# hassony2/handobjectconsist

Hardware: AMD Instinct MI355X
Metric: trainmeshwarp iters/sec (render+warp, B=64, 256x256) (higher is better)
Workload: dtype f32; 1 GPU; trainmeshwarp.py consist step, per-GPU B=64, 256x256, hand 778v/1552f + object 1002v/2000f (7104 faces after fill-back), ResNet-18 fp32 (MIOpen convolutions, channels-last, + fused HIP BatchNorm/ReLU/residual/max-pool kernels), Adam; global_batch=64, image_size=256, parallelism=dp1

## Files before the change

handobjectconsist_amd/csrc/stem_wrw.hip:

```cpp
#include "bn_device.hpp"

namespace mr {

constexpr int SW_TY = 4, SW_TX = 32;
constexpr int SW_BLOCKS = 512;
constexpr int SW_C = 64;
constexpr int SW_TAPS = 7 * 7 * 3;
constexpr int SW_NB = 5;
constexpr int SW_OUT = SW_C * SW_TAPS;
constexpr int SW_PH = 2 * SW_TY + 5;
constexpr int SW_PROW = (2 * SW_TX + 5) * 3;
constexpr int SW_PW = 213;
constexpr int SW_G = SW_TY * SW_TX * SW_C;
constexpr int SW_LDS = SW_G + SW_PH * SW_PW;
constexpr int SW_FIN_RUNS = 8, SW_FIN_RUN = SW_BLOCKS / SW_FIN_RUNS;
static_assert(SW_LDS >= SW_C * SW_NB * 32, "the wave reduction reuses the tile's LDS");
static_assert(SW_OUT % 32 == 0, "finish kernel: 32 outputs per workgroup");

typedef float f32x16 __attribute__((ext_vector_type(16)));

struct WrwParams {
    const float* grad_y;
    const float* grad_y2;
    const float* rec_d;
    const unsigned char* rec_code;
    BnAffine bn;
    const float* image;
    float* partial;
    int N, Hin, Win, H, W, OH, OW;
    int tiles_x, tiles_y;
    int64_t tiles;
};

__device__ __forceinline__ void wrw_keep(float& v) { asm volatile("" : "+v"(v)); }
__device__ __forceinline__ void wrw_keep(unsigned& v) { asm volatile("" : "+v"(v)); }
__device__ __forceinline__ void wrw_keep(float4& v) { asm volatile("" : "+v"(v.x), "+v"(v.y), "+v"(v.z), "+v"(v.w)); }

__global__ __launch_bounds__(256, 2) void stem_conv_wrw_kernel(WrwParams p) {
    __shared__ __attribute__((aligned(16))) float lds[SW_LDS];
    float* const G = lds;
    float* const patch = lds + SW_G;
    const int tid = threadIdx.x, lane = tid & 63, wave = tid >> 6, half = lane >> 5, l31 = lane & 31;

    const int c0 = 4 * (tid & 15), qcol = tid >> 4;
    float a[4], b[4];
#pragma unroll
    for (int i = 0; i < 4; i++) {
        float mean;
        channel_consts(p.bn, c0 + i, mean, a[i], b[i]);
    }

    const float* aptr[2];
    const float* bptr[SW_NB];
#pragma unroll
    for (int m = 0; m < 2; m++) aptr[m] = G + (wave * SW_TX + 16 * half) * SW_C + ((l31 + 32 * m) ^ (32 * half));
#pragma unroll
    for (int n = 0; n < SW_NB; n++) {
        const int t = l31 + 32 * n;
        const int off = t < SW_TAPS ? (t / 21) * SW_PW + t % 21 : 0;
        bptr[n] = patch + 2 * wave * SW_PW + 6 * 16 * half + off;
    }

    f32x16 acc[2][SW_NB];
#pragma unroll
    for (int m = 0; m < 2; m++)
#pragma unroll
        for (int n = 0; n < SW_NB; n++)
#pragma unroll
            for (int r = 0; r < 16; r++) acc[m][n][r] = 0.0f;

    const int per_image = p.tiles_x * p.tiles_y;
    for (int64_t tile = blockIdx.x; tile < p.tiles; tile += gridDim.x) {
        const int n = (int)(tile / per_image), rem = (int)(tile - (int64_t)n * per_image);
        const int cy0 = (rem / p.tiles_x) * SW_TY, cx0 = (rem % p.tiles_x) * SW_TX;

        {
            const int iy0 = 2 * cy0 - 3, ix0 = 2 * cx0 - 3;
            const int c = tid < SW_PROW ? tid : SW_PROW - 1, ix = ix0 + c / 3;
            const bool col = ix >= 0 && ix < p.Win;
            const float* src = p.image + (int64_t)n * p.Hin * p.Win * 3 + (col ? ix0 * 3 + c : 0);
            float pv[SW_PH];
#pragma unroll
            for (int r = 0; r < SW_PH; r++) {
                const int iy = iy0 + r, iyc = iy < 0 ? 0 : (iy >= p.Hin ? p.Hin - 1 : iy);
                pv[r] = src[(int64_t)iyc * p.Win * 3];
            }
#pragma unroll
            for (int r = 0; r < SW_PH; r++) wrw_keep(pv[r]);
#pragma unroll
            for (int r = 0; r < SW_PH; r++) {
                const int iy = iy0 + r;
                if (!col || iy < 0 || iy >= p.Hin) pv[r] = 0.0f;
            }
            if (tid < SW_PROW) {
#pragma unroll
                for (int r = 0; r < SW_PH; r++) patch[r * SW_PW + tid] = pv[r];
            }
        }

#pragma unroll 1
        for (int qr = 0; qr < SW_TY / 2; qr++) {
            float s[2][2][4];
            unsigned code[2][2][4];
            unsigned idw[2][2];
            float4 dv[2][2], g1[2][2], g2[2][2];
#pragma unroll
            for (int j = 0; j < 2; j++)
#pragma unroll
                for (int k = 0; k < 2; k++) {
                    const int wy = (cy0 >> 1) + qr + j, wx = (cx0 >> 1) + qcol + k;
                    const int64_t o = (((int64_t)n * p.OH + (wy < p.OH ? wy : p.OH - 1)) * p.OW + (wx < p.OW ? wx : p.OW - 1)) * SW_C + c0;
                    idw[j][k] = *reinterpret_cast<const unsigned*>(p.rec_code + o);
                    dv[j][k] = *reinterpret_cast<const float4*>(p.rec_d + o);
                    g1[j][k] = *reinterpret_cast<const float4*>(p.grad_y + o);
                    g2[j][k] = *reinterpret_cast<const float4*>((p.grad_y2 ? p.grad_y2 : p.grad_y) + o);
                }
#pragma unroll
            for (int j = 0; j < 2; j++)
#pragma unroll
                for (int k = 0; k < 2; k++) { wrw_keep(idw[j][k]); wrw_keep(dv[j][k]); wrw_keep(g1[j][k]); wrw_keep(g2[j][k]); }
#pragma unroll
            for (int j = 0; j < 2; j++)
#pragma unroll
                for (int k = 0; k < 2; k++) {
                    const int wy = (cy0 >> 1) + qr + j, wx = (cx0 >> 1) + qcol + k;
                    const bool win = wy < p.OH && wx < p.OW;
                    const float d[4] = {dv[j][k].x, dv[j][k].y, dv[j][k].z, dv[j][k].w};
                    const float gv[4] = {p.grad_y2 ? g1[j][k].x + g2[j][k].x : g1[j][k].x, p.grad_y2 ? g1[j][k].y + g2[j][k].y : g1[j][k].y,
                                         p.grad_y2 ? g1[j][k].z + g2[j][k].z : g1[j][k].z, p.grad_y2 ? g1[j][k].w + g2[j][k].w : g1[j][k].w};
#pragma unroll
                    for (int i = 0; i < 4; i++) {
                        code[j][k][i] = win ? (idw[j][k] >> (8 * i)) & 255u : 255u;
                        s[j][k][i] = (d[i] * a[i] + b[i] > 0.0f) ? gv[i] : 0.0f;
                    }
                }
#pragma unroll
            for (int pr = 0; pr < 2; pr++)
#pragma unroll
                for (int pc = 0; pc < 2; pc++) {
                    const int py = 2 * qr + pr, px = 2 * qcol + pc;
                    float g[4] = {0.0f, 0.0f, 0.0f, 0.0f};
#pragma unroll
                    for (int dy = 0; dy < 2; dy++) {
                        const int j = pr - dy, kh = pr + 1 - 2 * j;
                        if (j < 0) continue;
#pragma unroll
                        for (int dx = 0; dx < 2; dx++) {
                            const int k = pc - dx, kw = pc + 1 - 2 * k;
                            if (k < 0) continue;
                            const unsigned want = (unsigned)(kh * 3 + kw);
#pragma unroll
                            for (int i = 0; i < 4; i++) g[i] += code[j][k][i] == want ? s[j][k][i] : 0.0f;
                        }
                    }
                    const bool in = cy0 + py < p.H && cx0 + px < p.W;
                    float4 out;
                    out.x = in ? g[0] * a[0] : 0.0f; out.y = in ? g[1] * a[1] : 0.0f;
                    out.z = in ? g[2] * a[2] : 0.0f; out.w = in ? g[3] * a[3] : 0.0f;
                    *reinterpret_cast<float4*>(G + (py * SW_TX + px) * SW_C + (c0 ^ (((px >> 4) & 1) << 5))) = out;
                }
        }
        __syncthreads();

#pragma unroll
        for (int s = 0; s < 16; s++) {
            float av[2], bv[SW_NB];
#pragma unroll
            for (int m = 0; m < 2; m++) av[m] = aptr[m][s * SW_C];
#pragma unroll
            for (int nb = 0; nb < SW_NB; nb++) bv[nb] = bptr[nb][6 * s];
#pragma unroll
            for (int m = 0; m < 2; m++)
#pragma unroll
                for (int nb = 0; nb < SW_NB; nb++)
                    acc[m][nb] = __builtin_amdgcn_mfma_f32_32x32x2f32(av[m], bv[nb], acc[m][nb], 0, 0, 0);
        }
        __syncthreads();
    }

#pragma unroll 1
    for (int w = 0; w < 4; w++) {
        if (wave == w) {
#pragma unroll
            for (int m = 0; m < 2; m++)
#pragma unroll
                for (int nb = 0; nb < SW_NB; nb++)
#pragma unroll
                    for (int r = 0; r < 16; r++) {
                        float* const slot = lds + ((m * SW_NB + nb) * 16 + r) * 64 + lane;
                        *slot = w > 0 ? *slot + acc[m][nb][r] : acc[m][nb][r];
                    }
        }
        __syncthreads();
    }
    float* const out = p.partial + (int64_t)blockIdx.x * SW_OUT;
    for (int e = tid; e < 2 * SW_NB * 16 * 64; e += 256) {
        const int ln = e & 63, r = (e >> 6) & 15, blk = e >> 10, m = blk / SW_NB, nb = blk - m * SW_NB;
        const int c = 32 * m + (r & 3) + 8 * (r >> 2) + 4 * (ln >> 5), t = 32 * nb + (ln & 31);
        if (t < SW_TAPS) out[c * SW_TAPS + t] = lds[e];
    }
}

__global__ __launch_bounds__(256) void stem_conv_wrw_finish_kernel(const float* __restrict__ partial, float* __restrict__ out,
                                                                  int channels_last) {
    __shared__ double red[SW_FIN_RUNS][32];
    const int e = blockIdx.x * 32 + (threadIdx.x & 31), run = threadIdx.x >> 5;
    double v = 0.0;
    for (int j = 0; j < SW_FIN_RUN; j++) v += (double)partial[(int64_t)(run * SW_FIN_RUN + j) * SW_OUT + e];
    red[run][threadIdx.x & 31] = v;
    __syncthreads();
    if (threadIdx.x < 32) {
        double t = red[0][threadIdx.x];
#pragma unroll
        for (int r = 1; r < SW_FIN_RUNS; r++) t += red[r][threadIdx.x];
        const int c = e / SW_TAPS, tap = e - c * SW_TAPS;
        const int ci = tap % 3, k = tap / 3;
        out[channels_last ? e : c * SW_TAPS + ci * 49 + k] = (float)t;
    }
}

static bool wrw_geometry(WrwParams& p, int N, int C, int Hin, int Win) {
    if (N < 0 || Hin < 0 || Win < 0 || C != SW_C) return false;
    p.N = N; p.Hin = Hin; p.Win = Win;
    p.H = Hin > 0 ? (Hin - 1) / 2 + 1 : 0;
    p.W = Win > 0 ? (Win - 1) / 2 + 1 : 0;
    p.OH = p.H > 0 ? (p.H - 1) / 2 + 1 : 0;
    p.OW = p.W > 0 ? (p.W - 1) / 2 + 1 : 0;
    p.tiles_x = (p.W + SW_TX - 1) / SW_TX;
    p.tiles_y = (p.H + SW_TY - 1) / SW_TY;
    p.tiles = (int64_t)N * p.tiles_x * p.tiles_y;
    return true;
}

}

extern "C" int mr_stem_conv_wrw_tiling(int* tile_height, int* tile_width, int* workgroups) {
    if (tile_height) *tile_height = mr::SW_TY;
    if (tile_width) *tile_width = mr::SW_TX;
    if (workgroups) *workgroups = mr::SW_BLOCKS;
    return MR_OK;
}

extern "C" int64_t mr_stem_conv_wrw_workspace_bytes(int batch_size, int channels, int in_height, int in_width) {
    mr::WrwParams p{};
    if (!mr::wrw_geometry(p, batch_size, channels, in_height, in_width)) return -1;
    return (int64_t)mr::SW_BLOCKS * mr::SW_OUT * 4;
}

extern "C" int mr_stem_conv_wrw(const float* grad_y, const float* grad_y2, const unsigned char* records, const float* weight,
                                const float* bias, const float* running_mean, const float* running_var, float eps,
                                const float* image, float* grad_conv_weight, int weight_channels_last, void* workspace,
                                int64_t workspace_bytes, int batch_size, int channels, int in_height, int in_width,
                                int in_channels, int kernel_size, int stride, int padding, mr_stream_t stream) {
    using namespace mr;
    if (kernel_size != 7 || stride != 2 || padding != 3 || in_channels != 3) return MR_ERR_BADARG;
    WrwParams p{};
    if (!wrw_geometry(p, batch_size, channels, in_height, in_width)) return MR_ERR_BADARG;
    if (!grad_conv_weight) return MR_ERR_BADARG;
    const hipStream_t s = (hipStream_t)stream;
    if (p.tiles == 0) return zero_param_grads({grad_conv_weight}, SW_OUT, s);
    if (!grad_y || !records || !weight || !bias || !running_mean || !running_var || !image) return MR_ERR_BADARG;
    if (!workspace || workspace_bytes < mr_stem_conv_wrw_workspace_bytes(batch_size, channels, in_height, in_width)) return MR_ERR_BADARG;
    if (misaligned({records, grad_y, grad_y2}, 15) || misaligned({image, workspace, grad_conv_weight}, 3))
        return MR_ERR_BADARG;
    p.grad_y = grad_y; p.grad_y2 = grad_y2;
    p.rec_d = reinterpret_cast<const float*>(records);
    p.rec_code = records + (int64_t)p.N * p.OH * p.OW * SW_C * 4;
    p.bn = bn_affine(weight, bias, running_mean, running_var, eps);
    p.image = image;
    p.partial = static_cast<float*>(workspace);
    hipLaunchKernelGGL(stem_conv_wrw_kernel, dim3(SW_BLOCKS), dim3(256), 0, s, p);
    MR_CHECK_LAUNCH();
    hipLaunchKernelGGL(stem_conv_wrw_finish_kernel, dim3(SW_OUT / 32), dim3(256), 0, s, p.partial, grad_conv_weight,
                       weight_channels_last ? 1 : 0);
    MR_CHECK_LAUNCH();
    return MR_OK;
}
```

Before: 38.82 iters/s (one optimiser step = 1 data batch + 1 consist batch of B per GPU; roofline.stock_trunk_it_s = the same step with the trunk's BatchNorm/ReLU/max-pool on the stock nn modules).

## Pipeline stem weight-grad kernel with 16x16 MFMA tiles and prefetched next tile

Rewrites the stem conv weight-gradient kernel so each wave owns a disjoint channel/tap output tile using 16x16x4 MFMAs. This removes the cross-wave LDS reduction at the end. Global loads for the next tile are issued before the current tile's MFMA loop, and LDS operands are software-prefetched one step ahead, with a new bank swizzle. It also templates on whether a second gradient exists to skip the redundant grad_y2 load. The cost is higher register pressure from holding the next tile's raw data and the extra sched barriers.

```diff
diff --git a/handobjectconsist_amd/csrc/stem_wrw.hip b/handobjectconsist_amd/csrc/stem_wrw.hip
--- a/handobjectconsist_amd/csrc/stem_wrw.hip
+++ b/handobjectconsist_amd/csrc/stem_wrw.hip
@@ -1,12 +1,15 @@
 #include "bn_device.hpp"
 
 namespace mr {
+
+typedef float f32x4 __attribute__((ext_vector_type(4)));
 
 constexpr int SW_TY = 4, SW_TX = 32;
 constexpr int SW_BLOCKS = 512;
 constexpr int SW_C = 64;
 constexpr int SW_TAPS = 7 * 7 * 3;
-constexpr int SW_NB = 5;
+constexpr int SW_WT = 5;
+constexpr int SW_KS = SW_TX / 4;
 constexpr int SW_OUT = SW_C * SW_TAPS;
 constexpr int SW_PH = 2 * SW_TY + 5;
 constexpr int SW_PROW = (2 * SW_TX + 5) * 3;
@@ -14,10 +17,9 @@
 constexpr int SW_G = SW_TY * SW_TX * SW_C;
 constexpr int SW_LDS = SW_G + SW_PH * SW_PW;
 constexpr int SW_FIN_RUNS = 8, SW_FIN_RUN = SW_BLOCKS / SW_FIN_RUNS;
-static_assert(SW_LDS >= SW_C * SW_NB * 32, "the wave reduction reuses the tile's LDS");
 static_assert(SW_OUT % 32 == 0, "finish kernel: 32 outputs per workgroup");
-
-typedef float f32x16 __attribute__((ext_vector_type(16)));
+static_assert(SW_KS == 8 && SW_C == 64, "the bank swizzle of G: four k-lanes, four groups of 16 channels");
+static_assert(SW_PW % 32 == 21, "the patch's bank map: tap t in bank t");
 
 struct WrwParams {
     const float* grad_y;
@@ -34,13 +36,141 @@
 
 __device__ __forceinline__ void wrw_keep(float& v) { asm volatile("" : "+v"(v)); }
 __device__ __forceinline__ void wrw_keep(unsigned& v) { asm volatile("" : "+v"(v)); }
-__device__ __forceinline__ void wrw_keep(float4& v) { asm volatile("" : "+v"(v.x), "+v"(v.y), "+v"(v.z), "+v"(v.w)); }
-
+__device__ __forceinline__ void wrw_keep(f32x4& v) { asm volatile("" : "+v"(v)); }
+
+struct WrwTile {
+    int n, cy0, cx0;
+};
+
+__device__ __forceinline__ WrwTile wrw_tile(const WrwParams& p, int64_t tile) {
+    const int per_image = p.tiles_x * p.tiles_y;
+    const int n = (int)(tile / per_image), rem = (int)(tile - (int64_t)n * per_image);
+    return {n, (rem / p.tiles_x) * SW_TY, (rem % p.tiles_x) * SW_TX};
+}
+
+constexpr int SW_WR = SW_TY / 2 + 1;
+
+struct WrwRaw {
+    float pv[SW_PH];
+    unsigned code[SW_WR][2];
+    f32x4 d[SW_WR][2], g1[SW_WR][2], g2[SW_WR][2];
+};
+
+template <bool TWO>
+__device__ __forceinline__ void wrw_issue(const WrwParams& p, const WrwTile t, int tid, int c0, int qcol, WrwRaw& raw) {
+    const int iy0 = 2 * t.cy0 - 3, ix0 = 2 * t.cx0 - 3;
+    const int c = tid < SW_PROW ? tid : SW_PROW - 1, ix = ix0 + c / 3;
+    const bool col = ix >= 0 && ix < p.Win;
+    const float* src = p.image + (int64_t)t.n * p.Hin * p.Win * 3 + (col ? ix0 * 3 + c : 0);
+#pragma unroll
+    for (int r = 0; r < SW_PH; r++) {
+        const int iy = iy0 + r, iyc = iy < 0 ? 0 : (iy >= p.Hin ? p.Hin - 1 : iy);
+        raw.pv[r] = src[(int64_t)iyc * p.Win * 3];
+    }
+#pragma unroll
+    for (int wr = 0; wr < SW_WR; wr++)
+#pragma unroll
+        for (int k = 0; k < 2; k++) {
+            const int wy = (t.cy0 >> 1) + wr, wx = (t.cx0 >> 1) + qcol + k;
+            const int64_t o = (((int64_t)t.n * p.OH + (wy < p.OH ? wy : p.OH - 1)) * p.OW + (wx < p.OW ? wx : p.OW - 1)) * SW_C + c0;
+            raw.code[wr][k] = *reinterpret_cast<const unsigned*>(p.rec_code + o);
+            raw.d[wr][k] = *reinterpret_cast<const f32x4*>(p.rec_d + o);
+            raw.g1[wr][k] = *reinterpret_cast<const f32x4*>(p.grad_y + o);
+            if (TWO) raw.g2[wr][k] = *reinterpret_cast<const f32x4*>(p.grad_y2 + o);
+        }
+}
+
+template <bool TWO>
+__device__ __forceinline__ void wrw_build(const WrwParams& p, const WrwTile t, int tid, int c0, int qcol, const float (&a)[4],
+                                          const float (&b)[4], WrwRaw& raw, float* G, float* patch) {
+    {
+        const int iy0 = 2 * t.cy0 - 3, ix0 = 2 * t.cx0 - 3;
+        const int c = tid < SW_PROW ? tid : SW_PROW - 1, ix = ix0 + c / 3;
+        const bool col = ix >= 0 && ix < p.Win;
+#pragma unroll
+        for (int r = 0; r < SW_PH; r++) wrw_keep(raw.pv[r]);
+        if (tid < SW_PROW) {
+#pragma unroll
+            for (int r = 0; r < SW_PH; r++) {
+                const int iy = iy0 + r;
+                patch[r * SW_PW + tid] = (!col || iy < 0 || iy >= p.Hin) ? 0.0f : raw.pv[r];
+            }
+        }
+    }
+#pragma unroll
+    for (int wr = 0; wr < SW_WR; wr++)
+#pragma unroll
+        for (int k = 0; k < 2; k++) {
+            wrw_keep(raw.code[wr][k]); wrw_keep(raw.d[wr][k]); wrw_keep(raw.g1[wr][k]);
+            if (TWO) wrw_keep(raw.g2[wr][k]);
+        }
+#pragma unroll
+    for (int qr = 0; qr < SW_TY / 2; qr++) {
+        float s[2][2][4];
+        unsigned code[2][2][4];
+#pragma unroll
+        for (int j = 0; j < 2; j++)
+#pragma unroll
+            for (int k = 0; k < 2; k++) {
+                const int wy = (t.cy0 >> 1) + qr + j, wx = (t.cx0 >> 1) + qcol + k;
+                const bool win = wy < p.OH && wx < p.OW;
+                const f32x4 dv = raw.d[qr + j][k], g1 = raw.g1[qr + j][k], g2 = TWO ? raw.g2[qr + j][k] : g1;
+                const float d[4] = {dv.x, dv.y, dv.z, dv.w};
+                const float gv[4] = {TWO ? g1.x + g2.x : g1.x, TWO ? g1.y + g2.y : g1.y, TWO ? g1.z + g2.z : g1.z,
+                                     TWO ? g1.w + g2.w : g1.w};
+#pragma unroll
+                for (int i = 0; i < 4; i++) {
+                    code[j][k][i] = win ? (raw.code[qr + j][k] >> (8 * i)) & 255u : 255u;
+                    s[j][k][i] = (d[i] * a[i] + b[i] > 0.0f) ? gv[i] : 0.0f;
+                }
+            }
+#pragma unroll
+        for (int pr = 0; pr < 2; pr++)
+#pragma unroll
+            for (int pc = 0; pc < 2; pc++) {
+                const int py = 2 * qr + pr, px = 2 * qcol + pc;
+                float g[4] = {0.0f, 0.0f, 0.0f, 0.0f};
+#pragma unroll
+                for (int dy = 0; dy < 2; dy++) {
+                    const int j = pr - dy, kh = pr + 1 - 2 * j;
+                    if (j < 0) continue;
+#pragma unroll
+                    for (int dx = 0; dx < 2; dx++) {
+                        const int k = pc - dx, kw = pc + 1 - 2 * k;
+                        if (k < 0) continue;
+                        const unsigned want = (unsigned)(kh * 3 + kw);
+#pragma unroll
+                        for (int i = 0; i < 4; i++) g[i] += code[j][k][i] == want ? s[j][k][i] : 0.0f;
+                    }
+                }
+                const bool in = t.cy0 + py < p.H && t.cx0 + px < p.W;
+                float4 out;
+                out.x = in ? g[0] * a[0] : 0.0f; out.y = in ? g[1] * a[1] : 0.0f;
+                out.z = in ? g[2] * a[2] : 0.0f; out.w = in ? g[3] * a[3] : 0.0f;
+                *reinterpret_cast<float4*>(G + (py * SW_TX + px) * SW_C + (c0 ^ (16 * (px >> 3)))) = out;
+            }
+    }
+}
+
+struct WrwOperands {
+    float av[2], bv[SW_WT];
+};
+
+__device__ __forceinline__ void wrw_operands(const float* lds, const unsigned (&aoff)[2], const unsigned (&boff)[SW_WT], int q,
+                                             WrwOperands& o) {
+    const int r = q / SW_KS, s = q % SW_KS;
+#pragma unroll
+    for (int m = 0; m < 2; m++) o.av[m] = lds[aoff[m] + (r * SW_TX + s) * SW_C];
+#pragma unroll
+    for (int n = 0; n < SW_WT; n++) o.bv[n] = lds[boff[n] + 2 * r * SW_PW + 6 * s];
+}
+
+template <bool TWO>
 __global__ __launch_bounds__(256, 2) void stem_conv_wrw_kernel(WrwParams p) {
     __shared__ __attribute__((aligned(16))) float lds[SW_LDS];
     float* const G = lds;
     float* const patch = lds + SW_G;
-    const int tid = threadIdx.x, lane = tid & 63, wave = tid >> 6, half = lane >> 5, l31 = lane & 31;
+    const int tid = threadIdx.x, lane = tid & 63, wave = tid >> 6;
 
     const int c0 = 4 * (tid & 15), qcol = tid >> 4;
     float a[4], b[4];
@@ -50,155 +180,83 @@
         channel_consts(p.bn, c0 + i, mean, a[i], b[i]);
     }
 
-    const float* aptr[2];
-    const float* bptr[SW_NB];
-#pragma unroll
-    for (int m = 0; m < 2; m++) aptr[m] = G + (wave * SW_TX + 16 * half) * SW_C + ((l31 + 32 * m) ^ (32 * half));
-#pragma unroll
-    for (int n = 0; n < SW_NB; n++) {
-        const int t = l31 + 32 * n;
-        const int off = t < SW_TAPS ? (t / 21) * SW_PW + t % 21 : 0;
-        bptr[n] = patch + 2 * wave * SW_PW + 6 * 16 * half + off;
-    }
-
-    f32x16 acc[2][SW_NB];
+    const int l15 = lane & 15, kq = lane >> 4, wc = wave & 1, wt = wave >> 1;
+    unsigned aoff[2], boff[SW_WT];
+#pragma unroll
+    for (int m = 0; m < 2; m++) {
+        aoff[m] = (unsigned)(8 * kq * SW_C + ((32 * wc + 16 * m + l15) ^ (16 * kq)));
+        wrw_keep(aoff[m]);
+    }
+#pragma unroll
+    for (int n = 0; n < SW_WT; n++) {
+        const int t = 80 * wt + 16 * n + l15;
+        const int off = t < SW_TAPS ? (t / 21) * SW_PW + t % 21 : t - 64;
+        boff[n] = (unsigned)(SW_G + 6 * 8 * kq + off);
+        wrw_keep(boff[n]);
+    }
+
+    f32x4 tot[2][SW_WT];
 #pragma unroll
     for (int m = 0; m < 2; m++)
 #pragma unroll
-        for (int n = 0; n < SW_NB; n++)
-#pragma unroll
-            for (int r = 0; r < 16; r++) acc[m][n][r] = 0.0f;
-
-    const int per_image = p.tiles_x * p.tiles_y;
-    for (int64_t tile = blockIdx.x; tile < p.tiles; tile += gridDim.x) {
-        const int n = (int)(tile / per_image), rem = (int)(tile - (int64_t)n * per_image);
-        const int cy0 = (rem / p.tiles_x) * SW_TY, cx0 = (rem % p.tiles_x) * SW_TX;
-
-        {
-            const int iy0 = 2 * cy0 - 3, ix0 = 2 * cx0 - 3;
-            const int c = tid < SW_PROW ? tid : SW_PROW - 1, ix = ix0 + c / 3;
-            const bool col = ix >= 0 && ix < p.Win;
-            const float* src = p.image + (int64_t)n * p.Hin * p.Win * 3 + (col ? ix0 * 3 + c : 0);
-            float pv[SW_PH];
-#pragma unroll
-            for (int r = 0; r < SW_PH; r++) {
-                const int iy = iy0 + r, iyc = iy < 0 ? 0 : (iy >= p.Hin ? p.Hin - 1 : iy);
-                pv[r] = src[(int64_t)iyc * p.Win * 3];
+        for (int n = 0; n < SW_WT; n++) tot[m][n] = f32x4{0.0f, 0.0f, 0.0f, 0.0f};
+
+    if ((int64_t)blockIdx.x < p.tiles) {
+        int64_t tile = blockIdx.x;
+        WrwTile cur = wrw_tile(p, tile);
+        WrwRaw raw;
+        wrw_issue<TWO>(p, cur, tid, c0, qcol, raw);
+        for (;;) {
+            wrw_build<TWO>(p, cur, tid, c0, qcol, a, b, raw, G, patch);
+            __syncthreads();
+
+            const int64_t ahead = tile + gridDim.x;
+            const bool more = ahead < p.tiles;
+            const WrwTile next = wrw_tile(p, more ? ahead : tile);
+            WrwOperands ops;
+            wrw_operands(lds, aoff, boff, 0, ops);
+            wrw_issue<TWO>(p, next, tid, c0, qcol, raw);
+            __builtin_amdgcn_sched_barrier(0);
+
+            f32x4 acc[2][SW_WT];
+#pragma unroll
+            for (int q = 0; q < SW_TY * SW_KS; q++) {
+                const int s = q % SW_KS;
+                WrwOperands nxt = ops;
+                if (q + 1 < SW_TY * SW_KS) wrw_operands(lds, aoff, boff, q + 1, nxt);
+                __builtin_amdgcn_sched_barrier(0);
+#pragma unroll
+                for (int m = 0; m < 2; m++)
+#pragma unroll
+                    for (int n = 0; n < SW_WT; n++)
+                        acc[m][n] = __builtin_amdgcn_mfma_f32_16x16x4f32(ops.av[m], ops.bv[n], s == 0 ? f32x4{0.0f, 0.0f, 0.0f, 0.0f} : acc[m][n],
+                                                                         0, 0, 0);
+                if (s == SW_KS - 1) {
+#pragma unroll
+                    for (int m = 0; m < 2; m++)
+#pragma unroll
+                        for (int n = 0; n < SW_WT; n++) tot[m][n] += acc[m][n];
+                }
+                __builtin_amdgcn_sched_barrier(0);
+                ops = nxt;
             }
-#pragma unroll
-            for (int r = 0; r < SW_PH; r++) wrw_keep(pv[r]);
-#pragma unroll
-            for (int r = 0; r < SW_PH; r++) {
-                const int iy = iy0 + r;
-                if (!col || iy < 0 || iy >= p.Hin) pv[r] = 0.0f;
-            }
-            if (tid < SW_PROW) {
-#pragma unroll
-                for (int r = 0; r < SW_PH; r++) patch[r * SW_PW + tid] = pv[r];
-            }
-        }
-
-#pragma unroll 1
-        for (int qr = 0; qr < SW_TY / 2; qr++) {
-            float s[2][2][4];
-            unsigned code[2][2][4];
-            unsigned idw[2][2];
-            float4 dv[2][2], g1[2][2], g2[2][2];
-#pragma unroll
-            for (int j = 0; j < 2; j++)
-#pragma unroll
-                for (int k = 0; k < 2; k++) {
-                    const int wy = (cy0 >> 1) + qr + j, wx = (cx0 >> 1) + qcol + k;
-                    const int64_t o = (((int64_t)n * p.OH + (wy < p.OH ? wy : p.OH - 1)) * p.OW + (wx < p.OW ? wx : p.OW - 1)) * SW_C + c0;
-                    idw[j][k] = *reinterpret_cast<const unsigned*>(p.rec_code + o);
-                    dv[j][k] = *reinterpret_cast<const float4*>(p.rec_d + o);
-                    g1[j][k] = *reinterpret_cast<const float4*>(p.grad_y + o);
-                    g2[j][k] = *reinterpret_cast<const float4*>((p.grad_y2 ? p.grad_y2 : p.grad_y) + o);
-                }
-#pragma unroll
-            for (int j = 0; j < 2; j++)
-#pragma unroll
-                for (int k = 0; k < 2; k++) { wrw_keep(idw[j][k]); wrw_keep(dv[j][k]); wrw_keep(g1[j][k]); wrw_keep(g2[j][k]); }
-#pragma unroll
-            for (int j = 0; j < 2; j++)
-#pragma unroll
-                for (int k = 0; k < 2; k++) {
-                    const int wy = (cy0 >> 1) + qr + j, wx = (cx0 >> 1) + qcol + k;
-                    const bool win = wy < p.OH && wx < p.OW;
-                    const float d[4] = {dv[j][k].x, dv[j][k].y, dv[j][k].z, dv[j][k].w};
-                    const float gv[4] = {p.grad_y2 ? g1[j][k].x + g2[j][k].x : g1[j][k].x, p.grad_y2 ? g1[j][k].y + g2[j][k].y : g1[j][k].y,
-                                         p.grad_y2 ? g1[j][k].z + g2[j][k].z : g1[j][k].z, p.grad_y2 ? g1[j][k].w + g2[j][k].w : g1[j][k].w};
-#pragma unroll
-                    for (int i = 0; i < 4; i++) {
-                        code[j][k][i] = win ? (idw[j][k] >> (8 * i)) & 255u : 255u;
-                        s[j][k][i] = (d[i] * a[i] + b[i] > 0.0f) ? gv[i] : 0.0f;
-                    }
-                }
-#pragma unroll
-            for (int pr = 0; pr < 2; pr++)
-#pragma unroll
-                for (int pc = 0; pc < 2; pc++) {
-                    const int py = 2 * qr + pr, px = 2 * qcol + pc;
-                    float g[4] = {0.0f, 0.0f, 0.0f, 0.0f};
-#pragma unroll
-                    for (int dy = 0; dy < 2; dy++) {
-                        const int j = pr - dy, kh = pr + 1 - 2 * j;
-                        if (j < 0) continue;
-#pragma unroll
-                        for (int dx = 0; dx < 2; dx++) {
-                            const int k = pc - dx, kw = pc + 1 - 2 * k;
-                            if (k < 0) continue;
-                            const unsigned want = (unsigned)(kh * 3 + kw);
-#pragma unroll
-                            for (int i = 0; i < 4; i++) g[i] += code[j][k][i] == want ? s[j][k][i] : 0.0f;
-                        }
-                    }
-                    const bool in = cy0 + py < p.H && cx0 + px < p.W;
-                    float4 out;
-                    out.x = in ? g[0] * a[0] : 0.0f; out.y = in ? g[1] * a[1] : 0.0f;
-                    out.z = in ? g[2] * a[2] : 0.0f; out.w = in ? g[3] * a[3] : 0.0f;
-                    *reinterpret_cast<float4*>(G + (py * SW_TX + px) * SW_C + (c0 ^ (((px >> 4) & 1) << 5))) = out;
-                }
-        }
-        __syncthreads();
-
-#pragma unroll
-        for (int s = 0; s < 16; s++) {
-            float av[2], bv[SW_NB];
-#pragma unroll
-            for (int m = 0; m < 2; m++) av[m] = aptr[m][s * SW_C];
-#pragma unroll
-            for (int nb = 0; nb < SW_NB; nb++) bv[nb] = bptr[nb][6 * s];
-#pragma unroll
-            for (int m = 0; m < 2; m++)
-#pragma unroll
-                for (int nb = 0; nb < SW_NB; nb++)
-                    acc[m][nb] = __builtin_amdgcn_mfma_f32_32x32x2f32(av[m], bv[nb], acc[m][nb], 0, 0, 0);
-        }
-        __syncthreads();
-    }
-
-#pragma unroll 1
-    for (int w = 0; w < 4; w++) {
-        if (wave == w) {
-#pragma unroll
-            for (int m = 0; m < 2; m++)
-#pragma unroll
-                for (int nb = 0; nb < SW_NB; nb++)
-#pragma unroll
-                    for (int r = 0; r < 16; r++) {
-                        float* const slot = lds + ((m * SW_NB + nb) * 16 + r) * 64 + lane;
-                        *slot = w > 0 ? *slot + acc[m][nb][r] : acc[m][nb][r];
-                    }
-        }
-        __syncthreads();
-    }
+            __syncthreads();
+            if (!more) break;
+            tile = ahead;
+            cur = next;
+        }
+    }
+
     float* const out = p.partial + (int64_t)blockIdx.x * SW_OUT;
-    for (int e = tid; e < 2 * SW_NB * 16 * 64; e += 256) {
-        const int ln = e & 63, r = (e >> 6) & 15, blk = e >> 10, m = blk / SW_NB, nb = blk - m * SW_NB;
-        const int c = 32 * m + (r & 3) + 8 * (r >> 2) + 4 * (ln >> 5), t = 32 * nb + (ln & 31);
-        if (t < SW_TAPS) out[c * SW_TAPS + t] = lds[e];
-    }
+#pragma unroll
+    for (int m = 0; m < 2; m++)
+#pragma unroll
+        for (int n = 0; n < SW_WT; n++) {
+            const int t = 80 * wt + 16 * n + l15;
+            if (t >= SW_TAPS) continue;
+#pragma unroll
+            for (int i = 0; i < 4; i++) out[(32 * wc + 16 * m + 4 * kq + i) * SW_TAPS + t] = tot[m][n][i];
+        }
 }
 
 __global__ __launch_bounds__(256) void stem_conv_wrw_finish_kernel(const float* __restrict__ partial, float* __restrict__ out,
@@ -269,7 +327,8 @@
     p.bn = bn_affine(weight, bias, running_mean, running_var, eps);
     p.image = image;
     p.partial = static_cast<float*>(workspace);
-    hipLaunchKernelGGL(stem_conv_wrw_kernel, dim3(SW_BLOCKS), dim3(256), 0, s, p);
+    if (grad_y2) hipLaunchKernelGGL(stem_conv_wrw_kernel<true>, dim3(SW_BLOCKS), dim3(256), 0, s, p);
+    else hipLaunchKernelGGL(stem_conv_wrw_kernel<false>, dim3(SW_BLOCKS), dim3(256), 0, s, p);
     MR_CHECK_LAUNCH();
     hipLaunchKernelGGL(stem_conv_wrw_finish_kernel, dim3(SW_OUT / 32), dim3(256), 0, s, p.partial, grad_conv_weight,
                        weight_channels_last ? 1 : 0);
```

Result: no change. 38.76 iters/s (one optimiser step = 1 data batch + 1 consist batch of B per GPU; roofline.stock_trunk_it_s = the same step with the trunk's BatchNorm/ReLU/max-pool on the stock nn modules) (-0.2%).
